# facebookresearch/jepa

Hardware: AMD Instinct MI355X
Metric: V-JEPA pretrain clips/sec (fwd+bwd+EMA) (higher is better)
Workload: dtype bf16; 1 GPU; V-JEPA pretrain step ViT-L/16 16x224x224, B=24/GPU, 2 multiblock masks (vitl16.yaml); global_batch=24, per_gpu_batch=24, parallelism=dp1, hw_queues=4

## Files before the change

### include/vjepa_hip.h

```cpp
#ifndef VJEPA_HIP_H
#define VJEPA_HIP_H

#include <stdint.h>

#ifdef __cplusplus
extern "C" {
#endif

typedef struct ihipStream_t* vj_stream_t;

int vj_abi_version(void);
const char* vj_last_error(void);

int vj_gather_rows(const void* src, void* dst, const int64_t* idx, int64_t B, int64_t K, int64_t row_bytes,
                   int64_t src_batch_stride_rows, vj_stream_t stream);
int vj_scatter_rows(const void* src, void* dst, const int64_t* idx, int64_t B, int64_t N, int64_t K,
                    int64_t row_bytes, vj_stream_t stream);
int vj_copy_rows(const void* src, void* dst, int64_t B, int64_t src_rows, int64_t src_off, int64_t dst_rows,
                 int64_t dst_off, int64_t n, int64_t D, vj_stream_t stream);

int vj_tubelet_pack(const float* clips, void* out_bf16, const int64_t* idx, int64_t B, int64_t C, int64_t T,
                    int64_t H, int64_t W, int64_t tubelet, int64_t patch, int64_t K, vj_stream_t stream);
int vj_add_pos(void* x_bf16, const float* pos, const int64_t* idx, int64_t B, int64_t K, int64_t D,
               vj_stream_t stream);
// ... 37 lines not shown
                                 int64_t colpart_rows, int flags, int* fused, vj_stream_t stream);
int vj_gemm_bf16_nt_splitk(const void* A, int64_t lda, const void* B, int64_t ldb, float* C, int64_t ldc, int64_t M,
                           int64_t N, int64_t K, float alpha, float beta, int flags, void* ws, int64_t ws_bytes,
                           vj_stream_t stream);
int vj_gemm_bf16_tn_splitk(const void* dY, int64_t ldy, const void* X, int64_t ldx, float* dW, int64_t ldw, int64_t T,
                           int64_t N1, int64_t N2, float alpha, float beta, void* ws, int64_t ws_bytes,
                           vj_stream_t stream);
typedef struct vj_tn_problem {
  const void* dY; int64_t ldy;
  const void* X;  int64_t ldx;
  float* dW;      int64_t ldw;
  int64_t N1, N2;
} vj_tn_problem_t;
int vj_gemm_bf16_tn_grouped(const vj_tn_problem_t* problems, int64_t n, int64_t T, float alpha, float beta, void* ws,
                            int64_t ws_bytes, vj_stream_t stream);
int vj_transpose_bf16(const void* in, void* out, int64_t M, int64_t N, int64_t ld_in, int64_t Mpad,
                      vj_stream_t stream);
int vj_transpose_multi(const void* desc, const void* blocks, int64_t n_blocks, vj_stream_t stream);
int64_t vj_transpose_colsum_ws_bytes(int64_t M, int64_t N);
int vj_transpose_colsum_bf16(const void* in, void* out, int64_t M, int64_t N, int64_t ld_in, int64_t Mpad,
                             float* colsum, float alpha, float beta, void* ws, int64_t ws_bytes, vj_stream_t stream);
int64_t vj_colsum_ws_bytes(int64_t N);
int vj_colsum_bf16(const void* in, int64_t M, int64_t N, int64_t ld, int64_t group, int64_t row_lo, int64_t row_hi,
                   float* out, float alpha, float beta, void* ws, int64_t ws_bytes, vj_stream_t stream);
int vj_reduce_partials(const float* part, float* out, int64_t P, int64_t N, float alpha, float beta,
                       vj_stream_t stream);
typedef struct vj_reduce_seg {
  const float* part;
  float* out;
  int64_t P, N, stride;
// ... 162 lines not shown
```

### jepa_amd/csrc/gemm8_tn.hip

```cpp
#include <type_traits>
#include "gemm_common.hpp"
#include "options.hpp"

namespace {

__device__ __attribute__((aligned(256))) bf16_t g_tn_zero_row[128];

typedef __attribute__((ext_vector_type(4))) short tn_s16x4_t;
typedef __attribute__((ext_vector_type(8))) short tn_s16x8_t;

__device__ __forceinline__ bf16x8_t tn_frag(const char* p) {
  const tn_s16x4_t lo = __builtin_amdgcn_ds_read_tr16_b64_v4i16((__attribute__((address_space(3))) tn_s16x4_t*)p);
  const tn_s16x4_t hi =
      __builtin_amdgcn_ds_read_tr16_b64_v4i16((__attribute__((address_space(3))) tn_s16x4_t*)(p + 16 * 256));
  const tn_s16x8_t w = {lo[0], lo[1], lo[2], lo[3], hi[0], hi[1], hi[2], hi[3]};
  return __builtin_bit_cast(bf16x8_t, w);
}

struct TnLane {
  int row0;
  int sc8;
};

__device__ __forceinline__ void tn_issue_part(const GemmArgs& p, int q, int64_t m0, int64_t n0, int kt0, char* smem,
                                              const TnLane& tl, int wave_u) {
  const int qq = q + 1;
  const int kind = qq & 3;
  const int t = qq >> 2;
  const int64_t tok0 = (int64_t)(kt0 + t) * 64;
  char* slot = smem + ((q + 8) & 7) * LDS_PART_BYTES;
  const bool isA = (kind == 0) || (kind == 3);
  const int half = (kind == 0 || kind == 1) ? 0 : 1;
  const int64_t cbase = (isA ? m0 : n0) + half * 128;
  const int lim = (int)((isA ? p.M : p.N) - cbase - 8);
  const int rel = tl.sc8 < lim ? tl.sc8 : lim;
  const unsigned ld = (unsigned)(isA ? p.lda : p.ldb);
  const bf16_t* base = (isA ? p.A + tok0 * p.lda : p.B + tok0 * p.ldb) + cbase;
  const int64_t left = p.K - 1 - tok0;
  const int last_row = left < 63 ? (int)left : 63;
#pragma unroll
  for (int j = 0; j < 2; j++) {
    const int row = tl.row0 + 32 * j;
    const int rowc = row < last_row ? row : last_row;
// ... 24 lines not shown
  dma16_sv(f.base[KIND], v0, slot);
  dma16_sv(f.base[KIND], v1, slot + 512 * 16);
  f.base[KIND] += f.step[isA ? 0 : 1];
}

#define TN_GROUP_MAX 4
struct TnGroupArgs {
  int n;
  int unit_end[TN_GROUP_MAX];
  GemmArgs g[TN_GROUP_MAX];
};
struct TnSingleArgs {
  GemmArgs g;
};

template <bool GROUPED>
__global__ __launch_bounds__(512) void gemm_tn_8phase_kernel(std::conditional_t<GROUPED, TnGroupArgs, TnSingleArgs> ga) {
  extern __shared__ __attribute__((aligned(16))) char smem[];
  const int tid = threadIdx.x, lane = tid & 63;
  const int wave_u = __builtin_amdgcn_readfirstlane(tid >> 6);
  const int wm = wave_u >> 2, wn = wave_u & 3;
  const bool late_group = wave_u >= 4;

  GemmArgs p;
  p.colpart = nullptr;
  p.lnf_rs = nullptr;
  p.lnf_c = nullptr;
  p.raster = 0;
  p.qscale = 0.f;
  p.qcols = 0;
  int logical_all;
  if constexpr (GROUPED) {
    const int l = xcd_logical(blockIdx.x, ga.unit_end[ga.n - 1]);
    int idx = 0;
#pragma unroll
    for (int i = 0; i + 1 < TN_GROUP_MAX; i++)
      if (i + 1 < ga.n && l >= ga.unit_end[i]) idx = i + 1;
    logical_all = l - (idx > 0 ? ga.unit_end[idx - 1] : 0);
    p = ga.g[idx];
  } else {
    p = ga.g;
    logical_all = xcd_logical(blockIdx.x, p.tiles_m * p.tiles_n * p.splitk);
  }
  const int ntile = p.tiles_m * p.tiles_n;
  const int slice = logical_all / ntile;
  int tm, tn;
  tile_of(logical_all - slice * ntile, p.tiles_m, p.tiles_n, tm, tn);
  const int64_t m0 = (int64_t)tm * 256, n0 = (int64_t)tn * 256;
  const int nk_all = (int)((p.K + 63) / 64);
  const int kt0 = slice * p.ktiles_per;
  const int nk = (kt0 + p.ktiles_per < nk_all ? kt0 + p.ktiles_per : nk_all) - kt0;
  const int last_part = 4 * nk - 2;

  f32x4_t acc[2][2][4][2];
#pragma unroll
  for (int a = 0; a < 2; a++)
#pragma unroll
    for (int b = 0; b < 2; b++)
#pragma unroll
      for (int i = 0; i < 4; i++)
#pragma unroll
        for (int j = 0; j < 2; j++) acc[a][b][i][j] = (f32x4_t){0.f, 0.f, 0.f, 0.f};
  bf16x8_t ra0[4][2], ra1[4][2], rb0[2][2], rb1[2][2];

  int a_off[4], b_off[2];
  {
    const int g = lane >> 4, jj = (lane & 15) >> 2, q4 = lane & 3;
// ... 52 lines not shown
      }
    }
  };
  using NF0 = std::integral_constant<int, 0>;
  using NF4 = std::integral_constant<int, 4>;
  using NF8 = std::integral_constant<int, 8>;

  TnFast fs;
  {
    const unsigned sa = (unsigned)p.lda * 128u, sb = (unsigned)p.ldb * 128u;
    fs.step[0] = sa;
    fs.step[1] = sb;
    fs.row32[0] = sa >> 1;
    fs.row32[1] = sb >> 1;
#pragma unroll
    for (int kind = 0; kind < 4; kind++) {
      const bool isA = (kind == 0) || (kind == 3);
      const int half = (kind == 0 || kind == 1) ? 0 : 1;
      const int64_t cbase = (isA ? m0 : n0) + half * 128;
      const int first = (kind == 0 || kind == 1) ? 2 : 1;
      const int64_t tok0 = (int64_t)(kt0 + first) * 64;
      fs.base[kind] = (const char*)((isA ? p.A + tok0 * p.lda : p.B + tok0 * p.ldb) + cbase);
      fs.lim[kind] = (int)((isA ? p.M : p.N) - cbase - 8);
    }
    fs.tail_tile = (p.K & 63) ? nk_all - 1 - kt0 : -1;
  }
  const unsigned rowoff_a = (unsigned)tl.row0 * (unsigned)p.lda * 2u, rowoff_b = (unsigned)tl.row0 * (unsigned)p.ldb * 2u;
  auto issue_loop = [&](auto kind_tag, int q, int tile) __attribute__((always_inline)) {
    constexpr int KIND = decltype(kind_tag)::value;
    if (tile != fs.tail_tile && fs.lim[KIND] >= 0) tn_issue_fast<KIND>(fs, q, smem, tl.sc8, rowoff_a, rowoff_b, wave_u);
    else tn_issue_part(p, q, m0, n0, kt0, smem, tl, wave_u);
  };

  tn_issue_part(p, -1, m0, n0, kt0, smem, tl, wave_u);
#pragma unroll
  for (int q = 0; q < 5; q++)
    if (q <= last_part) tn_issue_part(p, q, m0, n0, kt0, smem, tl, wave_u);
  wait_landed(-1);
  section_barrier();
  if (late_group) section_barrier();
  {
    const char* slot = smem + 7 * LDS_PART_BYTES;
#pragma unroll
    for (int i = 0; i < 4; i++)
#pragma unroll
      for (int ks = 0; ks < 2; ks++) ra0[i][ks] = tn_frag(slot + a_off[i] + ks * 32 * 256);
  }
  section_barrier();
  section_barrier();

  for (int t = 0; t < nk; t++) {
#pragma unroll
    for (int ph = 0; ph < 4; ph++) {
      const int q = 4 * t + ph;
      if (ph == 0) {
        const char* slot = smem + (q & 7) * LDS_PART_BYTES;
#pragma unroll
        for (int j = 0; j < 2; j++)
#pragma unroll
          for (int ks = 0; ks < 2; ks++) rb0[j][ks] = tn_frag(slot + b_off[j] + ks * 32 * 256);
      }
      if (q + 5 <= last_part) {
        if (ph == 0) issue_loop(std::integral_constant<int, 2>{}, q + 5, t + 1);
        else if (ph == 1) issue_loop(std::integral_constant<int, 3>{}, q + 5, t + 1);
        else if (ph == 2) issue_loop(std::integral_constant<int, 0>{}, q + 5, t + 2);
        else issue_loop(std::integral_constant<int, 1>{}, q + 5, t + 2);
        wait_vmcnt<6>();
      } else {
        wait_landed(q);
      }
      section_barrier();
      const char* nslot = smem + ((q + 1) & 7) * LDS_PART_BYTES;
      if (ph == 0) {
        mma_rd(acc[0][0], rb0, ra0, NF4{}, [&](int f) { rb1[f >> 1][f & 1] = tn_frag(nslot + b_off[f >> 1] + (f & 1) * 32 * 256); });
      } else if (ph == 1) {
        mma_rd(acc[0][1], rb1, ra0, NF8{}, [&](int f) { ra1[f >> 1][f & 1] = tn_frag(nslot + a_off[f >> 1] + (f & 1) * 32 * 256); });
      } else if (ph == 2) {
        mma_rd(acc[1][1], rb1, ra1, NF8{}, [&](int f) { ra0[f >> 1][f & 1] = tn_frag(nslot + a_off[f >> 1] + (f & 1) * 32 * 256); });
      } else {
        mma_rd(acc[1][0], rb0, ra1, NF0{}, [&](int) {});
      }
      section_barrier();
    }
  }
  if (!late_group) section_barrier();

  const int elane = __builtin_amdgcn_mbcnt_hi(~0u, __builtin_amdgcn_mbcnt_lo(~0u, 0u));
  const int efrow = elane & 15, efg = elane >> 4;
#pragma unroll
  for (int ih = 0; ih < 2; ih++)
#pragma unroll
    for (int jh = 0; jh < 2; jh++)
      gemm_epilogue<EPI_F32, 4, 2, true>(p, acc[ih][jh], m0 + ih * 128 + wm * 64, n0 + jh * 128 + wn * 32, efrow, efg,
                                         slice);
}

}

static int tn_check(const char* who, const void* dY, int64_t ldy, const void* X, int64_t ldx, const float* dW, int64_t ldw,
                    int64_t T, int64_t N1, int64_t N2) {
  VJ_CHECK_ARG(T > 0, "%s: T must be positive", who);
  VJ_CHECK_ARG(N1 % 8 == 0 && N2 % 8 == 0, "%s: N1=%ld, N2=%ld must be multiples of 8", who, (long)N1, (long)N2);
  VJ_CHECK_ARG(ldy % 8 == 0 && ldx % 8 == 0 && ldy >= N1 && ldx >= N2 && ldy < (1 << 24) && ldx < (1 << 24),
               "%s: ldy/ldx must be multiples of 8, >= N1/N2 and < 2^24", who);
  VJ_CHECK_ARG(((uintptr_t)dY % 16 == 0) && ((uintptr_t)X % 16 == 0) && ((uintptr_t)dW % 16 == 0),
               "%s: operands must be 16-byte aligned", who);
  VJ_CHECK_ARG(ldw % 4 == 0 && ldw >= N2, "%s: ldw=%ld must be a multiple of 4 and >= N2", who, (long)ldw);
  return 0;
}

static GemmArgs tn_args(const void* dY, int64_t ldy, const void* X, int64_t ldx, float* dW, int64_t ldw, int64_t T,
// ... 5 lines not shown
  b.tiles_m = (int)cdiv64(N1, 256);
  b.tiles_n = (int)cdiv64(N2, 256);
  b.ktiles_per = (int)cdiv64(T, 64);
  return b;
}

template <bool GROUPED>
static void tn_set_attr() {
  static VjPerDeviceOnce attr_once;
  attr_once([] {
    (void)hipFuncSetAttribute((const void*)gemm_tn_8phase_kernel<GROUPED>, hipFuncAttributeMaxDynamicSharedMemorySize,
                              8 * LDS_PART_BYTES);
  });
}

extern "C" int vj_gemm_bf16_tn_splitk(const void* dY, int64_t ldy, const void* X, int64_t ldx, float* dW, int64_t ldw,
                                      int64_t T, int64_t N1, int64_t N2, float alpha, float beta, void* ws,
                                      int64_t ws_bytes, hipStream_t stream) {
  VJ_CHECK_ARG(T >= 0 && N1 >= 0 && N2 >= 0, "vj_gemm_bf16_tn_splitk: negative dim");
  if (N1 == 0 || N2 == 0) return 0;
  if (int rc = tn_check("vj_gemm_bf16_tn_splitk", dY, ldy, X, ldx, dW, ldw, T, N1, N2)) return rc;
  VJ_CHECK_ARG(ws != nullptr && ws_bytes >= N1 * N2 * 4, "vj_gemm_bf16_tn_splitk: workspace must hold at least N1*N2 fp32");
  tn_set_attr<false>();
  TnSingleArgs a;
  GemmArgs& b = a.g;
  b = tn_args(dY, ldy, X, ldx, dW, ldw, T, N1, N2, alpha, beta);
  const int nk = (int)cdiv64(T, 64);
  b.splitk = pick_splitk((int64_t)b.tiles_m * b.tiles_n, nk, 256, 1.45, 8, N1, N2, ws_bytes);
  b.ws = (float*)ws;
  vj_splitk_finish_plan(nk, b.splitk, b.ktiles_per);
  hipLaunchKernelGGL(gemm_tn_8phase_kernel<false>, dim3(b.tiles_m * b.tiles_n * b.splitk), dim3(512), 8 * LDS_PART_BYTES, stream, a);
  VJ_LAUNCH_CHECK("vj_gemm_bf16_tn_splitk");
  return vj_splitk_reduce(b, stream);
}

struct vj_tn_problem_abi {
  const void* dY; int64_t ldy;
  const void* X; int64_t ldx;
  float* dW; int64_t ldw;
  int64_t N1, N2;
};
extern "C" int vj_gemm_bf16_tn_grouped(const void* probs_v, int64_t n, int64_t T, float alpha, float beta, void* ws,
                                       int64_t ws_bytes, hipStream_t stream) {
  const vj_tn_problem_abi* pr = (const vj_tn_problem_abi*)probs_v;
  VJ_CHECK_ARG(n >= 0 && n <= TN_GROUP_MAX, "vj_gemm_bf16_tn_grouped: n=%ld (at most %d problems)", (long)n, TN_GROUP_MAX);
  VJ_CHECK_ARG(T >= 0, "vj_gemm_bf16_tn_grouped: negative T");
  TnGroupArgs a;
  a.n = 0;
  int64_t tiles = 0, out_elems = 0;
  for (int64_t i = 0; i < n; i++) {
    VJ_CHECK_ARG(pr[i].N1 >= 0 && pr[i].N2 >= 0, "vj_gemm_bf16_tn_grouped: negative dim");
    if (pr[i].N1 == 0 || pr[i].N2 == 0) continue;
    if (int rc = tn_check("vj_gemm_bf16_tn_grouped", pr[i].dY, pr[i].ldy, pr[i].X, pr[i].ldx, pr[i].dW, pr[i].ldw, T, pr[i].N1,
                          pr[i].N2))
      return rc;
    a.g[a.n] = tn_args(pr[i].dY, pr[i].ldy, pr[i].X, pr[i].ldx, pr[i].dW, pr[i].ldw, T, pr[i].N1, pr[i].N2, alpha, beta);
    tiles += (int64_t)a.g[a.n].tiles_m * a.g[a.n].tiles_n;
    out_elems += pr[i].N1 * pr[i].N2;
    a.n++;
  }
  if (a.n == 0) return 0;
  VJ_CHECK_ARG(ws != nullptr && ws_bytes >= out_elems * 4, "vj_gemm_bf16_tn_grouped: workspace must hold at least sum N1*N2 fp32");
  const int nk = (int)cdiv64(T, 64);
  int splitk = pick_splitk(tiles, nk, 256, 1.45, 8, out_elems, 1, ws_bytes);
  int ktiles_per;
  vj_splitk_finish_plan(nk, splitk, ktiles_per);
  int64_t units = 0, ws_off = 0;
  for (int i = 0; i < a.n; i++) {
    a.g[i].splitk = splitk;
    a.g[i].ktiles_per = ktiles_per;
    a.g[i].ws = (float*)((char*)ws + ws_off);
    ws_off += (int64_t)splitk * a.g[i].M * a.g[i].N * 4;
    units += (int64_t)a.g[i].tiles_m * a.g[i].tiles_n * splitk;
    a.unit_end[i] = (int)units;
  }
  for (int i = a.n; i < TN_GROUP_MAX; i++) {
    a.unit_end[i] = (int)units;
    a.g[i] = a.g[a.n - 1];
  }
  VJ_CHECK_ARG(units < (1ll << 31), "vj_gemm_bf16_tn_grouped: grid too large");
  tn_set_attr<true>();
  hipLaunchKernelGGL(gemm_tn_8phase_kernel<true>, dim3((unsigned)units), dim3(512), 8 * LDS_PART_BYTES, stream, a);
  VJ_LAUNCH_CHECK("vj_gemm_bf16_tn_grouped");
  for (int i = 0; i < a.n; i++)
    if (int rc = vj_splitk_reduce(a.g[i], stream)) return rc;
  return 0;
}
```

### jepa_amd/csrc/options.cpp

```cpp
#include "options.hpp"
#include <atomic>
#include <cstdlib>
#include <cstring>
#include <cctype>
#include <mutex>
#include <string>
#include "common.hpp"

namespace {
struct OptDef {
  const char* name;
  int dflt, lo, hi;
};
bool in_set(int id, int v) {
  if (id == VJ_OPT_GEMM_EPI_PRE) return v == 0 || v == 4;
  return true;
}
const OptDef kDefs[VJ_OPT_COUNT] = {
    {"gemm_fwd_flags", 0, 0, 0x1ff}, {"gemm_dgrad_flags", 0, 0, 0x1ff}, {"gemm_4w", 0, 0, 1},     {"gemm_persist", 2, 0, 3},
    {"wgrad_tn", 1, 0, 1},           {"wgrad_group", 1, 0, 1},          {"gemm_dbg", 0, 0, 7},    {"attn_softmax", 2, 1, 2},
    {"bias_fuse", 1, 0, 1},          {"gemm_raster", 260, 0, 511},      {"ws_guard", 0, 0, 1},    {"gemm_epi_pre", 4, 0, 4},
};
std::atomic<int> g_val[VJ_OPT_COUNT];
std::once_flag g_once;

void init_once() {
  std::call_once(g_once, [] {
    for (int i = 0; i < VJ_OPT_COUNT; i++) {
      std::string env = "VJ_";
      for (const char* c = kDefs[i].name; *c; c++) env.push_back((char)toupper((unsigned char)*c));
      const char* e = getenv(env.c_str());
      int v = e ? atoi(e) : kDefs[i].dflt;
      if (v < kDefs[i].lo || v > kDefs[i].hi || !in_set(i, v)) {
        fprintf(stderr, "libvjepa_hip: %s=%d outside [%d, %d], using the default %d\n", env.c_str(), v, kDefs[i].lo,
                kDefs[i].hi, kDefs[i].dflt);
// ... 38 lines not shown
```

### jepa_amd/hip/lib.py

```python
import ctypes
import os

import torch

_HERE = os.path.dirname(os.path.abspath(__file__))
_VARIANT = os.environ.get("VJ_LIB_VARIANT", "")
_LIB_PATH = os.path.join(os.path.dirname(_HERE), "lib", f"libvjepa_hip_{_VARIANT}.so" if _VARIANT else "libvjepa_hip.so")

P = ctypes.c_void_p
I64 = ctypes.c_int64
I32 = ctypes.c_int
F32 = ctypes.c_float
F64 = ctypes.c_double



class VjLinear(ctypes.Structure):
    _fields_ = [("w", P), ("b", P), ("wT", P), ("ldwT", I64), ("gw", P), ("gb", P), ("n_out", I64), ("k_in", I64)]


class VjNorm(ctypes.Structure):
    _fields_ = [("g", P), ("b", P), ("gg", P), ("gb", P)]


# ... 30 lines not shown
    "vj_image_pack": (I32, [P, P, P, I64, I64, I64, I64, I64, I64, I64, P]),
    "vj_add_pos_bcast": (I32, [P, P, P, I64, I64, I64, I64, P]),
    "vj_pos_interp3d": (I32, [P, P, I64, I64, I64, I64, F64, F64, F64, I64, I64, I64, P]),
    "vj_pos_interp2d_bicubic": (I32, [P, P, I64, I64, I64, F64, I64, I64, P]),
    "vj_add_pos_frames": (I32, [P, P, P, I64, I64, I64, I64, I64, P]),
    "vj_layernorm_fwd": (I32, [P, P, P, P, P, P, I64, I64, F32, P]),
    "vj_layernorm_bwd_ws_bytes": (I64, [I64]),
    "vj_layernorm_bwd": (I32, [P, P, P, P, P, P, P, P, P, F32, F32, I64, I64, P, I64, P]),
    "vj_layernorm_bwd_colsum": (I32, [P, P, P, P, P, P, P, P, P, P, F32, F32, I64, I64, P, I64, P]),
    "vj_gemm_bf16_nt": (I32, [P, I64, P, I64, P, I64, I64, I64, I64, P, P, I64, P, P, I64, I32, F32, F32, I32, P]),
    "vj_gemm_colsum_rows": (I64, [I64]),
    "vj_gemm_bf16_nt_dgelu_colsum": (I32, [P, I64, P, I64, P, I64, I64, I64, I64, P, I64, P, I64, I32, ctypes.POINTER(I32), P]),
    "vj_gemm_bf16_nt_splitk": (I32, [P, I64, P, I64, P, I64, I64, I64, I64, F32, F32, I32, P, I64, P]),
    "vj_gemm_bf16_tn_splitk": (I32, [P, I64, P, I64, P, I64, I64, I64, I64, F32, F32, P, I64, P]),
    "vj_gemm_bf16_tn_grouped": (I32, [P, I64, I64, F32, F32, P, I64, P]),
    "vj_transpose_bf16": (I32, [P, P, I64, I64, I64, I64, P]),
    "vj_transpose_multi": (I32, [P, P, I64, P]),
    "vj_transpose_colsum_ws_bytes": (I64, [I64, I64]),
    "vj_transpose_colsum_bf16": (I32, [P, P, I64, I64, I64, I64, P, F32, F32, P, I64, P]),
    "vj_colsum_ws_bytes": (I64, [I64]),
    "vj_colsum_bf16": (I32, [P, I64, I64, I64, I64, I64, I64, P, F32, F32, P, I64, P]),
    "vj_reduce_partials": (I32, [P, P, I64, I64, F32, F32, P]),
    "vj_reduce_segments": (I32, [P, I64, F32, F32, P]),
    "vj_attn_fwd": (I32, [P, P, P, I64, I64, I64, I64, F32, P]),
    "vj_attn_fwd_segs": (I32, [P, P, P, ctypes.POINTER(VjSeg), I64, I64, I64, F32, P]),
    "vj_attn_bwd_segs": (I32, [P, P, P, P, P, ctypes.POINTER(VjSeg), I64, I64, I64, F32, P, I64, P, P, P]),
    "vj_attn_bwd_ws_bytes": (I64, [I64, I64, I64]),
    "vj_attn_bwd_segs_ws_bytes": (I64, [ctypes.POINTER(VjSeg), I64, I64, I64]),
    "vj_attn_bwd": (I32, [P, P, P, P, P, I64, I64, I64, I64, F32, P, I64, P]),
    "vj_attn_bwd_colsum_rows": (I32, [I64, I64, I64, I64P, I64P]),
# ... 104 lines not shown
```

### jepa_amd/hip/ops.py

```python
import ctypes

import torch

from .lib import check, load_library

BF16 = torch.bfloat16
F32 = torch.float32
I64 = torch.int64

EPI_BF16, EPI_GELU, EPI_DGELU, EPI_F32 = 0, 1, 2, 3
EPI_QKV = 4


_raw_stream = torch._C._cuda_getCurrentRawStream
_dev_index = None


def _stream(stream=None):
    global _dev_index
    if stream is not None:
        return ctypes.c_void_p(stream)
    if _dev_index is None:
        _dev_index = torch.cuda.current_device()
    return ctypes.c_void_p(_raw_stream(_dev_index))
# ... 303 lines not shown
    lib = load_library()
    T = problems[0][0].shape[0]
    flat = []
    for dy, x, out in problems:
        _req(dy, BF16, "dy")
        _req(x, BF16, "x")
        assert dy.shape[0] == T and x.shape[0] == T and out.shape == (dy.shape[1], x.shape[1]) and out.dtype == F32
        flat += [dy.data_ptr(), dy.stride(0), x.data_ptr(), x.stride(0), out.data_ptr(), out.stride(0), dy.shape[1], x.shape[1]]
    arr = (ctypes.c_int64 * len(flat))(*[int(v) for v in flat])
    ws = Scratch.get(GROUP_WS_BYTES, problems[0][0].device, "wgrad_group", stream=stream)
    _ev = _timed("gemm_nt", sum(2.0 * T * dy.shape[1] * x.shape[1] for dy, x, _ in problems))
    check(lib.vj_gemm_bf16_tn_grouped(ctypes.addressof(arr), len(problems), T, alpha, beta, _ptr(ws), GROUP_WS_BYTES,
                                      _stream(stream)), "vj_gemm_bf16_tn_grouped")
    if _ev is not None:
        _ev.record()


def gemm_wgrad_tn(dy, x, out, alpha=1.0, beta=0.0, stream=None):
    lib = load_library()
    _req(dy, BF16, "dy")
    _req(x, BF16, "x")
    T, N1 = dy.shape
    N2 = x.shape[1]
    ws = Scratch.get(WGRAD_WS_BYTES, dy.device, "wgrad", stream=stream)
    _ev = _timed("gemm_nt", 2.0 * T * N1 * N2)
    check(lib.vj_gemm_bf16_tn_splitk(_ptr(dy), dy.stride(0), _ptr(x), x.stride(0), _ptr(out), out.stride(0), T, N1, N2,
                                     alpha, beta, _ptr(ws), WGRAD_WS_BYTES, _stream(stream)), "vj_gemm_bf16_tn_splitk")
    if _ev is not None:
        _ev.record()
    return out
# ... 322 lines not shown
```

Before: 333.7 clips/s.

## Split wgrad TN GEMM into partial-tile regions with cost-balanced split-K scheduling

Partitions each weight-gradient output into regions of full 256x256 tiles and half-width or quarter tiles at ragged edges. Specialized kernel variants skip loading and multiplying the empty A/B halves. A cost model assigns per-region split-K counts so the unit kernel balances work across CUs, followed by a multi-region reduce kernel. This removes wasted MFMA and load work on edge tiles, at the cost of an extra reduce launch, more template instantiations and a heuristic planner that may misbalance.

```diff
diff --git a/include/vjepa_hip.h b/include/vjepa_hip.h
--- a/include/vjepa_hip.h
+++ b/include/vjepa_hip.h
@@ -75,6 +75,8 @@
 } vj_tn_problem_t;
 int vj_gemm_bf16_tn_grouped(const vj_tn_problem_t* problems, int64_t n, int64_t T, float alpha, float beta, void* ws,
                             int64_t ws_bytes, vj_stream_t stream);
+int64_t vj_tn_plan_query(const int64_t* dims, int64_t n, int64_t T, int64_t slots, int64_t ws_bytes, int64_t form, int64_t* out,
+                         int64_t max_entries, int64_t* ws_need, int64_t* uses_kinds);
 int vj_transpose_bf16(const void* in, void* out, int64_t M, int64_t N, int64_t ld_in, int64_t Mpad,
                       vj_stream_t stream);
 int vj_transpose_multi(const void* desc, const void* blocks, int64_t n_blocks, vj_stream_t stream);
diff --git a/jepa_amd/csrc/gemm8_tn.hip b/jepa_amd/csrc/gemm8_tn.hip
--- a/jepa_amd/csrc/gemm8_tn.hip
+++ b/jepa_amd/csrc/gemm8_tn.hip
@@ -22,11 +22,26 @@
   int sc8;
 };
 
+enum { TN_FULL = 0, TN_NO_A1 = 1, TN_NO_B1 = 2, TN_QUARTER = 3 };
+template <int UK>
+struct TnKind {
+  static constexpr bool A1 = (UK == TN_FULL || UK == TN_NO_B1), B1 = (UK == TN_FULL || UK == TN_NO_A1);
+  static constexpr int NP = 2 + (A1 ? 1 : 0) + (B1 ? 1 : 0);
+  static constexpr int part(int j) { return (j == 2 && !B1) ? 3 : j; }
+};
+
+template <int UK>
 __device__ __forceinline__ void tn_issue_part(const GemmArgs& p, int q, int64_t m0, int64_t n0, int kt0, char* smem,
                                               const TnLane& tl, int wave_u) {
   const int qq = q + 1;
-  const int kind = qq & 3;
-  const int t = qq >> 2;
+  int kind, t;
+  if constexpr (TnKind<UK>::NP == 4) {
+    kind = qq & 3;
+    t = qq >> 2;
+  } else {
+    t = (int)((unsigned)qq / (unsigned)TnKind<UK>::NP);
+    kind = TnKind<UK>::part(qq - t * TnKind<UK>::NP);
+  }
   const int64_t tok0 = (int64_t)(kt0 + t) * 64;
   char* slot = smem + ((q + 8) & 7) * LDS_PART_BYTES;
   const bool isA = (kind == 0) || (kind == 3);
@@ -81,43 +96,16 @@
   GemmArgs g;
 };
 
-template <bool GROUPED>
-__global__ __launch_bounds__(512) void gemm_tn_8phase_kernel(std::conditional_t<GROUPED, TnGroupArgs, TnSingleArgs> ga) {
-  extern __shared__ __attribute__((aligned(16))) char smem[];
-  const int tid = threadIdx.x, lane = tid & 63;
-  const int wave_u = __builtin_amdgcn_readfirstlane(tid >> 6);
+template <int UK, bool REGION>
+__device__ __forceinline__ void tn_unit(const GemmArgs& p, const int64_t m0, const int64_t n0, const int kt0, const int nk,
+                                        const int slice, float* part, const int pitch, char* smem, const int tid,
+                                        const int wave_u) {
+  using KD = TnKind<UK>;
+  constexpr int NP = KD::NP;
+  const int lane = tid & 63;
   const int wm = wave_u >> 2, wn = wave_u & 3;
   const bool late_group = wave_u >= 4;
-
-  GemmArgs p;
-  p.colpart = nullptr;
-  p.lnf_rs = nullptr;
-  p.lnf_c = nullptr;
-  p.raster = 0;
-  p.qscale = 0.f;
-  p.qcols = 0;
-  int logical_all;
-  if constexpr (GROUPED) {
-    const int l = xcd_logical(blockIdx.x, ga.unit_end[ga.n - 1]);
-    int idx = 0;
-#pragma unroll
-    for (int i = 0; i + 1 < TN_GROUP_MAX; i++)
-      if (i + 1 < ga.n && l >= ga.unit_end[i]) idx = i + 1;
-    logical_all = l - (idx > 0 ? ga.unit_end[idx - 1] : 0);
-    p = ga.g[idx];
-  } else {
-    p = ga.g;
-    logical_all = xcd_logical(blockIdx.x, p.tiles_m * p.tiles_n * p.splitk);
-  }
-  const int ntile = p.tiles_m * p.tiles_n;
-  const int slice = logical_all / ntile;
-  int tm, tn;
-  tile_of(logical_all - slice * ntile, p.tiles_m, p.tiles_n, tm, tn);
-  const int64_t m0 = (int64_t)tm * 256, n0 = (int64_t)tn * 256;
-  const int nk_all = (int)((p.K + 63) / 64);
-  const int kt0 = slice * p.ktiles_per;
-  const int nk = (kt0 + p.ktiles_per < nk_all ? kt0 + p.ktiles_per : nk_all) - kt0;
-  const int last_part = 4 * nk - 2;
+  const int last_part = NP * nk - 2;
 
   f32x4_t acc[2][2][4][2];
 #pragma unroll
@@ -200,28 +188,30 @@
     fs.row32[0] = sa >> 1;
     fs.row32[1] = sb >> 1;
 #pragma unroll
-    for (int kind = 0; kind < 4; kind++) {
+    for (int j = 0; j < NP; j++) {
+      const int kind = KD::part(j);
       const bool isA = (kind == 0) || (kind == 3);
       const int half = (kind == 0 || kind == 1) ? 0 : 1;
       const int64_t cbase = (isA ? m0 : n0) + half * 128;
-      const int first = (kind == 0 || kind == 1) ? 2 : 1;
+      const int first = (6 - j + NP - 1) / NP;
       const int64_t tok0 = (int64_t)(kt0 + first) * 64;
       fs.base[kind] = (const char*)((isA ? p.A + tok0 * p.lda : p.B + tok0 * p.ldb) + cbase);
       fs.lim[kind] = (int)((isA ? p.M : p.N) - cbase - 8);
     }
+    const int nk_all = (int)((p.K + 63) / 64);
     fs.tail_tile = (p.K & 63) ? nk_all - 1 - kt0 : -1;
   }
   const unsigned rowoff_a = (unsigned)tl.row0 * (unsigned)p.lda * 2u, rowoff_b = (unsigned)tl.row0 * (unsigned)p.ldb * 2u;
   auto issue_loop = [&](auto kind_tag, int q, int tile) __attribute__((always_inline)) {
     constexpr int KIND = decltype(kind_tag)::value;
     if (tile != fs.tail_tile && fs.lim[KIND] >= 0) tn_issue_fast<KIND>(fs, q, smem, tl.sc8, rowoff_a, rowoff_b, wave_u);
-    else tn_issue_part(p, q, m0, n0, kt0, smem, tl, wave_u);
+    else tn_issue_part<UK>(p, q, m0, n0, kt0, smem, tl, wave_u);
   };
 
-  tn_issue_part(p, -1, m0, n0, kt0, smem, tl, wave_u);
+  tn_issue_part<UK>(p, -1, m0, n0, kt0, smem, tl, wave_u);
 #pragma unroll
   for (int q = 0; q < 5; q++)
-    if (q <= last_part) tn_issue_part(p, q, m0, n0, kt0, smem, tl, wave_u);
+    if (q <= last_part) tn_issue_part<UK>(p, q, m0, n0, kt0, smem, tl, wave_u);
   wait_landed(-1);
   section_barrier();
   if (late_group) section_barrier();
@@ -237,8 +227,8 @@
 
   for (int t = 0; t < nk; t++) {
 #pragma unroll
-    for (int ph = 0; ph < 4; ph++) {
-      const int q = 4 * t + ph;
+    for (int ph = 0; ph < NP; ph++) {
+      const int q = NP * t + ph;
       if (ph == 0) {
         const char* slot = smem + (q & 7) * LDS_PART_BYTES;
 #pragma unroll
@@ -247,24 +237,47 @@
           for (int ks = 0; ks < 2; ks++) rb0[j][ks] = tn_frag(slot + b_off[j] + ks * 32 * 256);
       }
       if (q + 5 <= last_part) {
-        if (ph == 0) issue_loop(std::integral_constant<int, 2>{}, q + 5, t + 1);
-        else if (ph == 1) issue_loop(std::integral_constant<int, 3>{}, q + 5, t + 1);
-        else if (ph == 2) issue_loop(std::integral_constant<int, 0>{}, q + 5, t + 2);
-        else issue_loop(std::integral_constant<int, 1>{}, q + 5, t + 2);
+        const int kind = KD::part((ph + 6) % NP), tile = t + (ph + 6) / NP;
+        if (kind == 2) issue_loop(std::integral_constant<int, 2>{}, q + 5, tile);
+        else if (kind == 3) issue_loop(std::integral_constant<int, 3>{}, q + 5, tile);
+        else if (kind == 0) issue_loop(std::integral_constant<int, 0>{}, q + 5, tile);
+        else issue_loop(std::integral_constant<int, 1>{}, q + 5, tile);
         wait_vmcnt<6>();
       } else {
         wait_landed(q);
       }
       section_barrier();
       const char* nslot = smem + ((q + 1) & 7) * LDS_PART_BYTES;
-      if (ph == 0) {
-        mma_rd(acc[0][0], rb0, ra0, NF4{}, [&](int f) { rb1[f >> 1][f & 1] = tn_frag(nslot + b_off[f >> 1] + (f & 1) * 32 * 256); });
-      } else if (ph == 1) {
-        mma_rd(acc[0][1], rb1, ra0, NF8{}, [&](int f) { ra1[f >> 1][f & 1] = tn_frag(nslot + a_off[f >> 1] + (f & 1) * 32 * 256); });
-      } else if (ph == 2) {
-        mma_rd(acc[1][1], rb1, ra1, NF8{}, [&](int f) { ra0[f >> 1][f & 1] = tn_frag(nslot + a_off[f >> 1] + (f & 1) * 32 * 256); });
+      if constexpr (UK == TN_FULL) {
+        if (ph == 0) {
+          mma_rd(acc[0][0], rb0, ra0, NF4{}, [&](int f) { rb1[f >> 1][f & 1] = tn_frag(nslot + b_off[f >> 1] + (f & 1) * 32 * 256); });
+        } else if (ph == 1) {
+          mma_rd(acc[0][1], rb1, ra0, NF8{}, [&](int f) { ra1[f >> 1][f & 1] = tn_frag(nslot + a_off[f >> 1] + (f & 1) * 32 * 256); });
+        } else if (ph == 2) {
+          mma_rd(acc[1][1], rb1, ra1, NF8{}, [&](int f) { ra0[f >> 1][f & 1] = tn_frag(nslot + a_off[f >> 1] + (f & 1) * 32 * 256); });
+        } else {
+          mma_rd(acc[1][0], rb0, ra1, NF0{}, [&](int) {});
+        }
+      } else if constexpr (UK == TN_NO_B1) {
+        if (ph == 0) {
+          mma_rd(acc[0][0], rb0, ra0, NF8{}, [&](int f) { ra1[f >> 1][f & 1] = tn_frag(nslot + a_off[f >> 1] + (f & 1) * 32 * 256); });
+        } else if (ph == 1) {
+          mma_rd(acc[1][0], rb0, ra1, NF8{}, [&](int f) { ra0[f >> 1][f & 1] = tn_frag(nslot + a_off[f >> 1] + (f & 1) * 32 * 256); });
+        }
       } else {
-        mma_rd(acc[1][0], rb0, ra1, NF0{}, [&](int) {});
+        if (ph == 0 && UK == TN_NO_A1) {
+          mma_rd(acc[0][0], rb0, ra0, NF4{}, [&](int f) { rb1[f >> 1][f & 1] = tn_frag(nslot + b_off[f >> 1] + (f & 1) * 32 * 256); });
+        } else if (ph == 0) {
+          mma_rd(acc[0][0], rb0, ra0, NF0{}, [&](int) {});
+        } else if (ph == 1 && UK == TN_NO_A1) {
+          mma_rd(acc[0][1], rb1, ra0, NF0{}, [&](int) {});
+        } else {
+          const char* slot = smem + (q & 7) * LDS_PART_BYTES;
+#pragma unroll
+          for (int i = 0; i < 4; i++)
+#pragma unroll
+            for (int ks = 0; ks < 2; ks++) ra0[i][ks] = tn_frag(slot + a_off[i] + ks * 32 * 256);
+        }
       }
       section_barrier();
     }
@@ -273,14 +286,299 @@
 
   const int elane = __builtin_amdgcn_mbcnt_hi(~0u, __builtin_amdgcn_mbcnt_lo(~0u, 0u));
   const int efrow = elane & 15, efg = elane >> 4;
-#pragma unroll
-  for (int ih = 0; ih < 2; ih++)
-#pragma unroll
-    for (int jh = 0; jh < 2; jh++)
-      gemm_epilogue<EPI_F32, 4, 2, true>(p, acc[ih][jh], m0 + ih * 128 + wm * 64, n0 + jh * 128 + wn * 32, efrow, efg,
-                                         slice);
-}
-
+  if constexpr (!REGION) {
+#pragma unroll
+    for (int ih = 0; ih < 2; ih++)
+#pragma unroll
+      for (int jh = 0; jh < 2; jh++)
+        gemm_epilogue<EPI_F32, 4, 2, true>(p, acc[ih][jh], m0 + ih * 128 + wm * 64, n0 + jh * 128 + wn * 32, efrow, efg,
+                                           slice);
+  } else {
+#pragma unroll
+    for (int ih = 0; ih < (KD::A1 ? 2 : 1); ih++)
+#pragma unroll
+      for (int jh = 0; jh < (KD::B1 ? 2 : 1); jh++) {
+        const int64_t mb = m0 + ih * 128 + wm * 64, nb = n0 + jh * 128 + wn * 32;
+        if (p.splitk > 1) {
+#pragma unroll
+          for (int i = 0; i < 4; i++) {
+            const int64_t m = mb + i * 16 + efrow;
+            float* row = part + m * pitch;
+#pragma unroll
+            for (int j = 0; j < 2; j++) {
+              const int64_t n = nb + j * 16 + efg * 4;
+              const f32x4_t v = acc[ih][jh][i][j];
+              if (m < p.M && n < p.N) *(float4*)(row + n) = make_float4(v[0], v[1], v[2], v[3]);
+            }
+          }
+        } else {
+          gemm_epilogue<EPI_F32, 4, 2, true>(p, acc[ih][jh], mb, nb, efrow, efg, slice);
+        }
+      }
+  }
+}
+
+template <bool GROUPED>
+__global__ __launch_bounds__(512) void gemm_tn_8phase_kernel(std::conditional_t<GROUPED, TnGroupArgs, TnSingleArgs> ga) {
+  extern __shared__ __attribute__((aligned(16))) char smem[];
+  const int tid = threadIdx.x;
+  const int wave_u = __builtin_amdgcn_readfirstlane(tid >> 6);
+
+  GemmArgs p;
+  p.colpart = nullptr;
+  p.lnf_rs = nullptr;
+  p.lnf_c = nullptr;
+  p.raster = 0;
+  p.qscale = 0.f;
+  p.qcols = 0;
+  int logical_all;
+  if constexpr (GROUPED) {
+    const int l = xcd_logical(blockIdx.x, ga.unit_end[ga.n - 1]);
+    int idx = 0;
+#pragma unroll
+    for (int i = 0; i + 1 < TN_GROUP_MAX; i++)
+      if (i + 1 < ga.n && l >= ga.unit_end[i]) idx = i + 1;
+    logical_all = l - (idx > 0 ? ga.unit_end[idx - 1] : 0);
+    p = ga.g[idx];
+  } else {
+    p = ga.g;
+    logical_all = xcd_logical(blockIdx.x, p.tiles_m * p.tiles_n * p.splitk);
+  }
+  const int ntile = p.tiles_m * p.tiles_n;
+  const int slice = logical_all / ntile;
+  int tm, tn;
+  tile_of(logical_all - slice * ntile, p.tiles_m, p.tiles_n, tm, tn);
+  const int64_t m0 = (int64_t)tm * 256, n0 = (int64_t)tn * 256;
+  const int nk_all = (int)((p.K + 63) / 64);
+  const int kt0 = slice * p.ktiles_per;
+  const int nk = (kt0 + p.ktiles_per < nk_all ? kt0 + p.ktiles_per : nk_all) - kt0;
+  tn_unit<TN_FULL, false>(p, m0, n0, kt0, nk, slice, nullptr, 0, smem, tid, wave_u);
+}
+
+#define TN_REGION_MAX (4 * TN_GROUP_MAX)
+#define TN_ENTRY_MAX (2 * TN_REGION_MAX)
+struct TnUnitRegion {
+  int prob, kind, tm0, tn0, ntm, ntn;
+  int splitk, ktiles_per;
+  int pitch;
+  int64_t plane;
+  float* ws;
+};
+struct TnUnitEntry {
+  int unit_end;
+  int region, slice0;
+};
+struct TnUnitArgs {
+  int n_entries;
+  TnUnitEntry e[TN_ENTRY_MAX];
+  TnUnitRegion r[TN_REGION_MAX];
+  GemmArgs g[TN_GROUP_MAX];
+};
+
+__global__ __launch_bounds__(512) void gemm_tn_units_kernel(TnUnitArgs ga) {
+  extern __shared__ __attribute__((aligned(16))) char smem[];
+  const int tid = threadIdx.x;
+  const int wave_u = __builtin_amdgcn_readfirstlane(tid >> 6);
+  const int l = xcd_logical(blockIdx.x, ga.e[ga.n_entries - 1].unit_end);
+  int idx = 0;
+#pragma unroll
+  for (int i = 0; i + 1 < TN_ENTRY_MAX; i++)
+    if (i + 1 < ga.n_entries && l >= ga.e[i].unit_end) idx = i + 1;
+  const TnUnitEntry en = ga.e[idx];
+  const int local = l - (idx > 0 ? ga.e[idx - 1].unit_end : 0);
+  const TnUnitRegion rg = ga.r[en.region];
+  GemmArgs p = ga.g[rg.prob];
+  p.colpart = nullptr;
+  p.lnf_rs = nullptr;
+  p.lnf_c = nullptr;
+  p.raster = 0;
+  p.qscale = 0.f;
+  p.qcols = 0;
+  p.splitk = rg.splitk;
+  p.ktiles_per = rg.ktiles_per;
+  const int ntile = rg.ntm * rg.ntn;
+  const int ds = local / ntile, tl = local - ds * ntile;
+  const int slice = en.slice0 + ds;
+  const int tnr = tl / rg.ntm, tmr = tl - tnr * rg.ntm;
+  const int64_t m0 = (int64_t)(rg.tm0 + tmr) * 256, n0 = (int64_t)(rg.tn0 + tnr) * 256;
+  const int nk_all = (int)((p.K + 63) / 64);
+  const int kt0 = slice * rg.ktiles_per;
+  const int nk = (kt0 + rg.ktiles_per < nk_all ? kt0 + rg.ktiles_per : nk_all) - kt0;
+  float* part = rg.ws + (int64_t)slice * rg.plane - ((int64_t)rg.tm0 * 256 * rg.pitch + (int64_t)rg.tn0 * 256);
+  const int kind = __builtin_amdgcn_readfirstlane(rg.kind);
+  if (kind == TN_FULL) tn_unit<TN_FULL, true>(p, m0, n0, kt0, nk, slice, part, rg.pitch, smem, tid, wave_u);
+  else if (kind == TN_NO_A1) tn_unit<TN_NO_A1, true>(p, m0, n0, kt0, nk, slice, part, rg.pitch, smem, tid, wave_u);
+  else if (kind == TN_NO_B1) tn_unit<TN_NO_B1, true>(p, m0, n0, kt0, nk, slice, part, rg.pitch, smem, tid, wave_u);
+  else tn_unit<TN_QUARTER, true>(p, m0, n0, kt0, nk, slice, part, rg.pitch, smem, tid, wave_u);
+}
+
+struct TnReduceArgs {
+  int n;
+  int blk_end[TN_REGION_MAX];
+  const float4* ws[TN_REGION_MAX];
+  float* out[TN_REGION_MAX];
+  int64_t ldc[TN_REGION_MAX];
+  int rows[TN_REGION_MAX], cols[TN_REGION_MAX], S[TN_REGION_MAX];
+};
+__global__ __launch_bounds__(256) void tn_reduce_regions_kernel(TnReduceArgs ra, float alpha, float beta) {
+  int sg = 0;
+  while (sg + 1 < ra.n && (int)blockIdx.x >= ra.blk_end[sg]) sg++;
+  const int blk0 = sg == 0 ? 0 : ra.blk_end[sg - 1], nblk = ra.blk_end[sg] - blk0;
+  const float4* __restrict__ ws = ra.ws[sg];
+  const int64_t nq = ra.cols[sg] / 4, n4 = (int64_t)ra.rows[sg] * nq;
+  const int S = ra.S[sg];
+  for (int64_t q = (int64_t)((int)blockIdx.x - blk0) * 256 + threadIdx.x; q < n4; q += (int64_t)nblk * 256) {
+    float4 acc = ws[q];
+    for (int s = 1; s < S; s++) {
+      const float4 v = ws[(int64_t)s * n4 + q];
+      acc.x += v.x;
+      acc.y += v.y;
+      acc.z += v.z;
+      acc.w += v.w;
+    }
+    const int64_t m = q / nq, n = (q - m * nq) * 4;
+    float* cp = ra.out[sg] + m * ra.ldc[sg] + n;
+    float4 o = make_float4(acc.x * alpha, acc.y * alpha, acc.z * alpha, acc.w * alpha);
+    if (beta != 0.f) {
+      const float4 c0 = *(const float4*)cp;
+      o.x += beta * c0.x;
+      o.y += beta * c0.y;
+      o.z += beta * c0.z;
+      o.w += beta * c0.w;
+    }
+    *(float4*)cp = o;
+  }
+}
+
+}
+
+static const double kTnKindCost[4] = {1.0, 0.75, 0.75, 0.60};
+#define TN_UNIT_OVERHEAD 4.0
+#define TN_US_PER_KTILE 1.45
+#define TN_MIN_KTILES 8
+#define TN_SLOTS 256
+
+struct TnPlanRegion {
+  int prob, kind, tm0, tn0, ntm, ntn, splitk, ktiles_per, rows, cols;
+  int64_t ws_off, ws_bytes;
+};
+struct TnPlanEntry {
+  int region, slice0, nslices, ktiles, unit_begin, unit_end;
+  double cost;
+};
+struct TnPlan {
+  int n_regions = 0, n_entries = 0, units = 0;
+  bool all_full = true;
+  int64_t ws_need = 0;
+  TnPlanRegion r[TN_REGION_MAX];
+  TnPlanEntry e[TN_ENTRY_MAX];
+};
+
+static void tn_plan_regions(TnPlan& pl, int prob, int64_t N1, int64_t N2) {
+  const int tiles_m = (int)cdiv64(N1, 256), tiles_n = (int)cdiv64(N2, 256);
+  const bool half_m = N1 - (int64_t)(tiles_m - 1) * 256 <= 128, half_n = N2 - (int64_t)(tiles_n - 1) * 256 <= 128;
+  const int fm = tiles_m - (half_m ? 1 : 0), fn = tiles_n - (half_n ? 1 : 0);
+  auto add = [&](int kind, int tm0, int tn0, int ntm, int ntn) {
+    if (ntm <= 0 || ntn <= 0) return;
+    TnPlanRegion& r = pl.r[pl.n_regions++];
+    r.prob = prob; r.kind = kind; r.tm0 = tm0; r.tn0 = tn0; r.ntm = ntm; r.ntn = ntn;
+    r.splitk = 1; r.ktiles_per = 0;
+    const int64_t r1 = (int64_t)(tm0 + ntm) * 256, c1 = (int64_t)(tn0 + ntn) * 256;
+    r.rows = (int)((r1 < N1 ? r1 : N1) - (int64_t)tm0 * 256);
+    r.cols = (int)((c1 < N2 ? c1 : N2) - (int64_t)tn0 * 256);
+    r.ws_off = r.ws_bytes = 0;
+    if (kind != TN_FULL) pl.all_full = false;
+  };
+  add(TN_FULL, 0, 0, fm, fn);
+  add(TN_NO_B1, 0, fn, fm, tiles_n - fn);
+  add(TN_NO_A1, fm, 0, tiles_m - fm, fn);
+  add(TN_QUARTER, fm, fn, tiles_m - fm, tiles_n - fn);
+}
+
+static void tn_plan_finish(TnPlan& pl, int nk, const int per[4]) {
+  pl.n_entries = 0;
+  int64_t off = 0;
+  for (int i = 0; i < pl.n_regions; i++) {
+    TnPlanRegion& r = pl.r[i];
+    r.ktiles_per = per[r.kind];
+    r.splitk = (nk + r.ktiles_per - 1) / r.ktiles_per;
+    r.ws_off = off;
+    r.ws_bytes = r.splitk > 1 ? (int64_t)r.splitk * r.rows * r.cols * 4 : 0;
+    off += r.ws_bytes;
+    const int tail = nk - (r.splitk - 1) * r.ktiles_per;
+    auto add = [&](int slice0, int nslices, int ktiles) {
+      TnPlanEntry& e = pl.e[pl.n_entries++];
+      e.region = i; e.slice0 = slice0; e.nslices = nslices; e.ktiles = ktiles;
+      e.cost = kTnKindCost[r.kind] * ktiles + TN_UNIT_OVERHEAD;
+    };
+    if (tail == r.ktiles_per) add(0, r.splitk, tail);
+    else {
+      add(0, r.splitk - 1, r.ktiles_per);
+      add(r.splitk - 1, 1, tail);
+    }
+  }
+  pl.ws_need = off;
+  for (int a = 1; a < pl.n_entries; a++) {
+    const TnPlanEntry x = pl.e[a];
+    int b = a;
+    for (; b > 0 && pl.e[b - 1].cost < x.cost; b--) pl.e[b] = pl.e[b - 1];
+    pl.e[b] = x;
+  }
+  int u = 0;
+  for (int a = 0; a < pl.n_entries; a++) {
+    TnPlanEntry& e = pl.e[a];
+    e.unit_begin = u;
+    u += e.nslices * pl.r[e.region].ntm * pl.r[e.region].ntn;
+    e.unit_end = u;
+  }
+  pl.units = u;
+}
+
+static void tn_plan_balanced(TnPlan& pl, int nk, int slots, int64_t ws_bytes) {
+  int64_t tiles[4] = {0, 0, 0, 0}, area[4] = {0, 0, 0, 0};
+  for (int i = 0; i < pl.n_regions; i++) {
+    tiles[pl.r[i].kind] += pl.r[i].ntm * pl.r[i].ntn;
+    area[pl.r[i].kind] += (int64_t)pl.r[i].rows * pl.r[i].cols;
+  }
+  const int per_min = nk < TN_MIN_KTILES ? nk : TN_MIN_KTILES;
+  const int per_floor = (nk + 63) / 64 > per_min ? (nk + 63) / 64 : per_min;
+  int best[4] = {nk, nk, nk, nk};
+  double best_cost = 1e30;
+  for (int ck = 0; ck < 4; ck++) {
+    if (!tiles[ck]) continue;
+    for (int cper = per_floor; cper <= nk; cper++) {
+      const double L = kTnKindCost[ck] * cper;
+      int per[4] = {nk, nk, nk, nk};
+      int64_t units = 0, ws = 0;
+      double longest = 0.0, partial_us = 0.0;
+      for (int k = 0; k < 4; k++) {
+        if (!tiles[k]) continue;
+        int pk = (int)(L / kTnKindCost[k] + 1e-9);
+        pk = pk < per_floor ? per_floor : pk > nk ? nk : pk;
+        const int s = (nk + pk - 1) / pk;
+        pk = (nk + s - 1) / s;
+        per[k] = pk;
+        units += tiles[k] * s;
+        if (s > 1) {
+          ws += (int64_t)s * area[k] * 4;
+          partial_us += 2.0 * (double)s * (double)area[k] * 4.0 / 3.0e6;
+        }
+        if (kTnKindCost[k] * pk > longest) longest = kTnKindCost[k] * pk;
+      }
+      if (ws > ws_bytes) continue;
+      const int64_t rounds = (units + slots - 1) / slots;
+      const double cost = (double)rounds * (longest + TN_UNIT_OVERHEAD) * TN_US_PER_KTILE + partial_us;
+      if (cost < best_cost) {
+        best_cost = cost;
+        for (int k = 0; k < 4; k++) best[k] = per[k];
+      }
+    }
+  }
+  tn_plan_finish(pl, nk, best);
+}
+static void tn_plan_uniform(TnPlan& pl, int nk, int ktiles_per) {
+  const int per[4] = {ktiles_per, ktiles_per, ktiles_per, ktiles_per};
+  tn_plan_finish(pl, nk, per);
 }
 
 static int tn_check(const char* who, const void* dY, int64_t ldy, const void* X, int64_t ldx, const float* dW, int64_t ldw,
@@ -316,6 +614,52 @@
   });
 }
 
+static int tn_launch_units(const char* who, const GemmArgs* g, int n, const TnPlan& pl, void* ws, hipStream_t stream) {
+  static VjPerDeviceOnce attr_once;
+  attr_once([] {
+    (void)hipFuncSetAttribute((const void*)gemm_tn_units_kernel, hipFuncAttributeMaxDynamicSharedMemorySize, 8 * LDS_PART_BYTES);
+  });
+  TnUnitArgs a;
+  TnReduceArgs ra;
+  ra.n = 0;
+  int nblk = 0;
+  for (int i = 0; i < TN_GROUP_MAX; i++) a.g[i] = g[i < n ? i : n - 1];
+  for (int i = 0; i < TN_REGION_MAX; i++) {
+    const TnPlanRegion& r = pl.r[i < pl.n_regions ? i : pl.n_regions - 1];
+    TnUnitRegion& d = a.r[i];
+    d.prob = r.prob; d.kind = r.kind;
+    d.tm0 = r.tm0; d.tn0 = r.tn0; d.ntm = r.ntm; d.ntn = r.ntn;
+    d.splitk = r.splitk; d.ktiles_per = r.ktiles_per;
+    d.pitch = r.cols;
+    d.plane = (int64_t)r.rows * r.cols;
+    d.ws = (float*)((char*)ws + r.ws_off);
+    if (i < pl.n_regions && r.splitk > 1) {
+      const GemmArgs& b = g[r.prob];
+      const int k = ra.n++;
+      ra.ws[k] = (const float4*)d.ws;
+      ra.out[k] = (float*)b.C + (int64_t)r.tm0 * 256 * b.ldc + (int64_t)r.tn0 * 256;
+      ra.ldc[k] = b.ldc;
+      ra.rows[k] = r.rows; ra.cols[k] = r.cols; ra.S[k] = r.splitk;
+      nblk += flat_grid((int64_t)r.rows * r.cols / 4, 256 * 8);
+      ra.blk_end[k] = nblk;
+    }
+  }
+  a.n_entries = pl.n_entries;
+  for (int i = 0; i < TN_ENTRY_MAX; i++) {
+    const TnPlanEntry& e = pl.e[i < pl.n_entries ? i : pl.n_entries - 1];
+    a.e[i].unit_end = e.unit_end;
+    a.e[i].region = e.region;
+    a.e[i].slice0 = e.slice0;
+  }
+  hipLaunchKernelGGL(gemm_tn_units_kernel, dim3((unsigned)pl.units), dim3(512), 8 * LDS_PART_BYTES, stream, a);
+  VJ_LAUNCH_CHECK(who);
+  if (ra.n > 0) {
+    hipLaunchKernelGGL(tn_reduce_regions_kernel, dim3((unsigned)nblk), dim3(256), 0, stream, ra, g[0].alpha, g[0].beta);
+    VJ_LAUNCH_CHECK("vj_gemm_bf16_tn(region reduce)");
+  }
+  return 0;
+}
+
 extern "C" int vj_gemm_bf16_tn_splitk(const void* dY, int64_t ldy, const void* X, int64_t ldx, float* dW, int64_t ldw,
                                       int64_t T, int64_t N1, int64_t N2, float alpha, float beta, void* ws,
                                       int64_t ws_bytes, hipStream_t stream) {
@@ -323,7 +667,6 @@
   if (N1 == 0 || N2 == 0) return 0;
   if (int rc = tn_check("vj_gemm_bf16_tn_splitk", dY, ldy, X, ldx, dW, ldw, T, N1, N2)) return rc;
   VJ_CHECK_ARG(ws != nullptr && ws_bytes >= N1 * N2 * 4, "vj_gemm_bf16_tn_splitk: workspace must hold at least N1*N2 fp32");
-  tn_set_attr<false>();
   TnSingleArgs a;
   GemmArgs& b = a.g;
   b = tn_args(dY, ldy, X, ldx, dW, ldw, T, N1, N2, alpha, beta);
@@ -331,6 +674,15 @@
   b.splitk = pick_splitk((int64_t)b.tiles_m * b.tiles_n, nk, 256, 1.45, 8, N1, N2, ws_bytes);
   b.ws = (float*)ws;
   vj_splitk_finish_plan(nk, b.splitk, b.ktiles_per);
+  if (vj_opt(VJ_OPT_WGRAD_GROUP) != 2) {
+    TnPlan pl;
+    tn_plan_regions(pl, 0, N1, N2);
+    if (!pl.all_full) {
+      tn_plan_uniform(pl, nk, b.ktiles_per);
+      return tn_launch_units("vj_gemm_bf16_tn_splitk", &b, 1, pl, ws, stream);
+    }
+  }
+  tn_set_attr<false>();
   hipLaunchKernelGGL(gemm_tn_8phase_kernel<false>, dim3(b.tiles_m * b.tiles_n * b.splitk), dim3(512), 8 * LDS_PART_BYTES, stream, a);
   VJ_LAUNCH_CHECK("vj_gemm_bf16_tn_splitk");
   return vj_splitk_reduce(b, stream);
@@ -348,6 +700,7 @@
   VJ_CHECK_ARG(n >= 0 && n <= TN_GROUP_MAX, "vj_gemm_bf16_tn_grouped: n=%ld (at most %d problems)", (long)n, TN_GROUP_MAX);
   VJ_CHECK_ARG(T >= 0, "vj_gemm_bf16_tn_grouped: negative T");
   TnGroupArgs a;
+  TnPlan pl;
   a.n = 0;
   int64_t tiles = 0, out_elems = 0;
   for (int64_t i = 0; i < n; i++) {
@@ -357,6 +710,7 @@
                           pr[i].N2))
       return rc;
     a.g[a.n] = tn_args(pr[i].dY, pr[i].ldy, pr[i].X, pr[i].ldx, pr[i].dW, pr[i].ldw, T, pr[i].N1, pr[i].N2, alpha, beta);
+    tn_plan_regions(pl, a.n, pr[i].N1, pr[i].N2);
     tiles += (int64_t)a.g[a.n].tiles_m * a.g[a.n].tiles_n;
     out_elems += pr[i].N1 * pr[i].N2;
     a.n++;
@@ -364,9 +718,17 @@
   if (a.n == 0) return 0;
   VJ_CHECK_ARG(ws != nullptr && ws_bytes >= out_elems * 4, "vj_gemm_bf16_tn_grouped: workspace must hold at least sum N1*N2 fp32");
   const int nk = (int)cdiv64(T, 64);
-  int splitk = pick_splitk(tiles, nk, 256, 1.45, 8, out_elems, 1, ws_bytes);
+  int splitk = pick_splitk(tiles, nk, TN_SLOTS, TN_US_PER_KTILE, TN_MIN_KTILES, out_elems, 1, ws_bytes);
   int ktiles_per;
   vj_splitk_finish_plan(nk, splitk, ktiles_per);
+  const int form = vj_opt(VJ_OPT_WGRAD_GROUP);
+  if (form != 2 && !pl.all_full) {
+    if (form == 3) tn_plan_uniform(pl, nk, ktiles_per);
+    else tn_plan_balanced(pl, nk, TN_SLOTS, ws_bytes);
+    VJ_CHECK_ARG(pl.ws_need <= ws_bytes, "vj_gemm_bf16_tn_grouped: the plan needs %ld workspace bytes, %ld given", (long)pl.ws_need,
+                 (long)ws_bytes);
+    return tn_launch_units("vj_gemm_bf16_tn_grouped", a.g, a.n, pl, ws, stream);
+  }
   int64_t units = 0, ws_off = 0;
   for (int i = 0; i < a.n; i++) {
     a.g[i].splitk = splitk;
@@ -388,3 +750,62 @@
     if (int rc = vj_splitk_reduce(a.g[i], stream)) return rc;
   return 0;
 }
+
+extern "C" int64_t vj_tn_plan_query(const int64_t* dims, int64_t n, int64_t T, int64_t slots, int64_t ws_bytes, int64_t form,
+                                    int64_t* out, int64_t max_entries, int64_t* ws_need, int64_t* uses_kinds) {
+  VJ_CHECK_ARG(dims != nullptr && out != nullptr && n >= 1 && n <= TN_GROUP_MAX && T > 0 && slots > 0, "vj_tn_plan_query: bad arguments");
+  TnPlan pl;
+  int64_t tiles = 0, out_elems = 0;
+  for (int i = 0; i < (int)n; i++) {
+    VJ_CHECK_ARG(dims[2 * i] > 0 && dims[2 * i + 1] > 0, "vj_tn_plan_query: bad dims");
+    tn_plan_regions(pl, i, dims[2 * i], dims[2 * i + 1]);
+    tiles += cdiv64(dims[2 * i], 256) * cdiv64(dims[2 * i + 1], 256);
+    out_elems += dims[2 * i] * dims[2 * i + 1];
+  }
+  const int nk = (int)cdiv64(T, 64);
+  int splitk = pick_splitk(tiles, nk, (int)slots, TN_US_PER_KTILE, TN_MIN_KTILES, out_elems, 1, ws_bytes);
+  int ktiles_per;
+  vj_splitk_finish_plan(nk, splitk, ktiles_per);
+  const bool kinds = form != 2 && !pl.all_full;
+  if (!kinds) {
+    pl = TnPlan();
+    for (int i = 0; i < (int)n; i++) {
+      TnPlanRegion& r = pl.r[pl.n_regions++];
+      r.prob = i; r.kind = TN_FULL; r.tm0 = r.tn0 = 0;
+      r.ntm = (int)cdiv64(dims[2 * i], 256); r.ntn = (int)cdiv64(dims[2 * i + 1], 256);
+      r.rows = (int)dims[2 * i]; r.cols = (int)dims[2 * i + 1];
+    }
+    tn_plan_uniform(pl, nk, ktiles_per);
+    int u = 0;
+    pl.n_entries = 0;
+    const int tail = nk - (splitk - 1) * ktiles_per;
+    for (int i = 0; i < pl.n_regions; i++)
+      for (int part = 0; part < 2; part++) {
+        const int nsl = part == 0 ? (tail == ktiles_per ? splitk : splitk - 1) : (tail == ktiles_per ? 0 : 1);
+        if (nsl == 0) continue;
+        TnPlanEntry& e = pl.e[pl.n_entries++];
+        e.region = i; e.slice0 = part == 0 ? 0 : splitk - 1; e.nslices = nsl; e.ktiles = part == 0 ? ktiles_per : tail;
+        e.cost = e.ktiles + TN_UNIT_OVERHEAD;
+        e.unit_begin = u;
+        u += nsl * pl.r[i].ntm * pl.r[i].ntn;
+        e.unit_end = u;
+      }
+    pl.units = u;
+  } else if (form == 3) {
+    tn_plan_uniform(pl, nk, ktiles_per);
+  } else {
+    tn_plan_balanced(pl, nk, (int)slots, ws_bytes);
+  }
+  VJ_CHECK_ARG(pl.n_entries <= max_entries, "vj_tn_plan_query: %d entries, room for %ld", pl.n_entries, (long)max_entries);
+  for (int i = 0; i < pl.n_entries; i++) {
+    const TnPlanEntry& e = pl.e[i];
+    const TnPlanRegion& r = pl.r[e.region];
+    int64_t* o = out + 16 * i;
+    o[0] = r.prob; o[1] = r.kind; o[2] = r.tm0; o[3] = r.tn0; o[4] = r.ntm; o[5] = r.ntn; o[6] = r.splitk; o[7] = r.ktiles_per;
+    o[8] = e.slice0; o[9] = e.nslices; o[10] = e.ktiles; o[11] = e.unit_begin; o[12] = e.unit_end; o[13] = r.ws_off; o[14] = r.ws_bytes;
+    o[15] = (int64_t)(e.cost * 1000.0 + 0.5);
+  }
+  if (ws_need) *ws_need = pl.ws_need;
+  if (uses_kinds) *uses_kinds = kinds ? 1 : 0;
+  return pl.n_entries;
+}
diff --git a/jepa_amd/csrc/options.cpp b/jepa_amd/csrc/options.cpp
--- a/jepa_amd/csrc/options.cpp
+++ b/jepa_amd/csrc/options.cpp
@@ -18,7 +18,7 @@
 }
 const OptDef kDefs[VJ_OPT_COUNT] = {
     {"gemm_fwd_flags", 0, 0, 0x1ff}, {"gemm_dgrad_flags", 0, 0, 0x1ff}, {"gemm_4w", 0, 0, 1},     {"gemm_persist", 2, 0, 3},
-    {"wgrad_tn", 1, 0, 1},           {"wgrad_group", 1, 0, 1},          {"gemm_dbg", 0, 0, 7},    {"attn_softmax", 2, 1, 2},
+    {"wgrad_tn", 1, 0, 1},           {"wgrad_group", 1, 0, 3},          {"gemm_dbg", 0, 0, 7},    {"attn_softmax", 2, 1, 2},
     {"bias_fuse", 1, 0, 1},          {"gemm_raster", 260, 0, 511},      {"ws_guard", 0, 0, 1},    {"gemm_epi_pre", 4, 0, 4},
 };
 std::atomic<int> g_val[VJ_OPT_COUNT];
diff --git a/jepa_amd/hip/lib.py b/jepa_amd/hip/lib.py
--- a/jepa_amd/hip/lib.py
+++ b/jepa_amd/hip/lib.py
@@ -68,6 +68,7 @@
     "vj_gemm_bf16_nt_splitk": (I32, [P, I64, P, I64, P, I64, I64, I64, I64, F32, F32, I32, P, I64, P]),
     "vj_gemm_bf16_tn_splitk": (I32, [P, I64, P, I64, P, I64, I64, I64, I64, F32, F32, P, I64, P]),
     "vj_gemm_bf16_tn_grouped": (I32, [P, I64, I64, F32, F32, P, I64, P]),
+    "vj_tn_plan_query": (I64, [I64P, I64, I64, I64, I64, I64, I64P, I64, I64P, I64P]),
     "vj_transpose_bf16": (I32, [P, P, I64, I64, I64, I64, P]),
     "vj_transpose_multi": (I32, [P, P, I64, P]),
     "vj_transpose_colsum_ws_bytes": (I64, [I64, I64]),
diff --git a/jepa_amd/hip/ops.py b/jepa_amd/hip/ops.py
--- a/jepa_amd/hip/ops.py
+++ b/jepa_amd/hip/ops.py
@@ -341,6 +341,21 @@
                                       _stream(stream)), "vj_gemm_bf16_tn_grouped")
     if _ev is not None:
         _ev.record()
+
+
+TN_PLAN_FIELDS = ("problem", "kind", "tm0", "tn0", "ntm", "ntn", "splitk", "ktiles_per", "slice0", "nslices", "ktiles", "unit_begin",
+                  "unit_end", "ws_off", "ws_bytes", "cost_milli")
+
+
+def tn_plan(dims, T, slots=256, ws_bytes=GROUP_WS_BYTES, form=1):
+    lib = load_library()
+    flat = (ctypes.c_int64 * (2 * len(dims)))(*[int(v) for d in dims for v in d])
+    out = (ctypes.c_int64 * (16 * 32))()
+    need, kinds = ctypes.c_int64(0), ctypes.c_int64(0)
+    n = lib.vj_tn_plan_query(flat, len(dims), T, slots, ws_bytes, form, out, 32, ctypes.byref(need), ctypes.byref(kinds))
+    if n < 0:
+        check(int(n), "vj_tn_plan_query")
+    return [dict(zip(TN_PLAN_FIELDS, out[16 * i:16 * i + 16])) for i in range(n)], int(need.value), bool(kinds.value)
 
 
 def gemm_wgrad_tn(dy, x, out, alpha=1.0, beta=0.0, stream=None):
```

After: 334.5 clips/s (median of 6 runs). No clear change (+0.2%).
